# vasudeva-ram/Julia-NewtonRaphsonHANK

Hardware: AMD Instinct MI355X
Metric: sequence-space JVPs/sec (household block: BackwardIteration+ForwardIteration+aggregation, Krusell-Smith T=300) (higher is better)
Workload: dtype f64; 1 GPU; ks_2000x11_T300_N32; grid=2000x11, T=300, tangents_per_gpu=32, step=1 dual-sweep pass: primal + N tangents (hank_primal_jvp), parallelism=tangent-sharded x1

## Files before the change

### julia-newtonraphsonhank_amd/csrc/hank_device.h

```cpp
#pragma once
#include <hip/hip_runtime.h>
#include <stdint.h>
#include "hank_geom.h"

#ifndef HANK_XFWD_LQ
#define HANK_XFWD_LQ 1
#endif
#ifndef HANK_XFWD_EARLY_BATCH
#define HANK_XFWD_EARLY_BATCH 0
#endif

namespace hank {

struct Consts {
    int n_a, n_e, G, P;
    int n_hh;
    int diet;
    double beta, gamma, bc;
    const double *a, *z, *Pi;
};

struct Record {
    double *s, *kc, *A, *B, *u, *v, *pol, *lw, *ig, *Dseq;
    int *ib, *lo, *start, *clo;
    int4 *seg;
    double2 *lwg;
};

__device__ inline double wave_sum(double x) {
#pragma unroll
    for (int off = 32; off > 0; off >>= 1) x += __shfl_down(x, off, 64);
    return x;
}
__device__ inline double block_sum(double x, double *red, int nthreads) {
    const int lane = threadIdx.x & 63, wv = threadIdx.x >> 6;
    const int nw = (nthreads + 63) >> 6;
    x = wave_sum(x);
    __syncthreads();
    if (lane == 0) red[wv] = x;
    __syncthreads();
    double r = 0.0;
    if (threadIdx.x == 0)
        for (int k = 0; k < nw; k++) r += red[k];
    return r;
}
// ... 719 lines not shown
```

### julia-newtonraphsonhank_amd/csrc/hank_hip.hip

```cpp
#include "hank_kernels.h"
#include "hank_xsweep.h"
#include "hank_xspec.h"
#include "hank_jacobian.h"
#include "hank_wide.h"
#include "hank_hetx.h"
#include "hank_scen.h"
#include "hank_ssbatch.h"
#include "hank_adjoint.h"
#include "hank_boundary.h"
#include "hank_ssdiff_launch.h"
#include "../../include/hank_hip.h"

#include <cstdarg>
#include <cstdio>
#include <cstdlib>
#include <cstring>
#include <initializer_list>
#include <list>
#include <mutex>
#include <new>
#include <vector>

using namespace hank;

// ... 55 lines not shown
    GraphExec &tan_fwd(bool bnd, int NX) { return g_tfwd[bnd][NX]; }
private:
    GraphExec g_tback[2], g_tfwd[2][3];
};

constexpr int XD_MAX = 4;
constexpr int XPASS_MAX = 64;
struct XPass { int n0, N, D, groups; size_t dpol_off; };
struct XTan {
    int N = 0;
    std::vector<XPass> passes;
    DevBuf<double> dxhh, dxr, dxw, dxt;
    DevBuf<double> dpol;
    DevBuf<double> daggpart;
    DevBuf<double> dagg_pass;
    DevBuf<double> dagg_cm;
};
struct XWork {
    bool ready = false;
    int grid = 0, Sact = 0, maxt = 768, dmax = XD_MAX;
    DevBuf<XSync> sync;
    DevBuf<double> st_s, st_ds, st_D, st_dD;
    DevBuf<double> Dvirt, aggpart, rho;
    DevBuf<double> D0own;
    DevBuf<int> srcB, srcF;
    DevBuf<int2> unitsF;
    DevBuf<int> unit_overflow;
    int ucap = 64;
    bool rng_valid = false;
    DevBuf<int2> stageU;
    DevBuf<int4> stageM;
    bool front = true;
    int front_poison = 0;
    bool neigh = true;
    bool syncwave = true;
    int lds_max = 65536;
    int fault_where = 7;
    int fault = 0;
    bool src_valid = false;
    std::list<XTan> tans;
    int last_blocks = 0;
    int xspec = XSPEC_CRRA;
    int inst[4] = {-1, -1, -1, -1};
};

struct WTan {
    int N = 0;
    DevBuf<double> dxhh;
    DevBuf<double> dpol;
    DevBuf<double> dagg_cm;
};

struct CotWork {
    int N = 0;
    int V = 1;
    AdjGeom g{};
    DevBuf<double> ybar;
    DevBuf<double> yb0, yb1;
    DevBuf<double> ybx;
    DevBuf<double> st[2];
    DevBuf<double> pbar;
    DevBuf<double> partS, partM;
    DevBuf<double> xbar;
    GraphExec g_A, g_B;
    GraphExec g_AX[2];
    DevBuf<double> bnd_vbar, bnd_dbar;
// ... 587 lines not shown

static int x_setup(hank_ctx *ctx) {
    XWork &X = ctx->xw;
    if (X.ready) return HANK_OK;
    const Consts &c = ctx->c;
    hipDeviceProp_t prop;
    HIPC(ctx, hipGetDeviceProperties(&prop, ctx->device));
    X.grid = (prop.multiProcessorCount / XG) * XG;
    X.Sact = (c.n_a + XRW - 1) / XRW;
    X.maxt = 64 * (c.n_e + 1) <= 768 ? 768 : 1024;
    X.dmax = X.maxt == 768 ? XD_MAX : 2;
    const size_t G = c.G, GV = G + 64 * (size_t)c.n_e, P = c.P;
    HIPC(ctx, X.sync.alloc((size_t)2 + 2 * XPASS_MAX));
    HIPC(ctx, hipMemsetAsync(X.sync, 0, sizeof(XSync) * ((size_t)2 + 2 * XPASS_MAX), ctx->stream));
    HIPC(ctx, X.st_s.alloc(2 * XG * G));
    HIPC(ctx, X.st_ds.alloc(2 * XG * G * X.dmax));
    const size_t GM = (size_t)c.n_e * X.Sact * 64;
    HIPC(ctx, X.st_D.alloc(2 * XG * std::max(GV, GM)));
    HIPC(ctx, X.st_dD.alloc(2 * XG * GM * xslots(X.dmax + 1).SP));
    HIPC(ctx, X.Dvirt.alloc(P * c.n_e * 64));
    HIPC(ctx, X.D0own.alloc(P * c.n_e));
    HIPC(ctx, X.aggpart.alloc(2 * P * (size_t)X.Sact));
    HIPC(ctx, X.rho.alloc(P));
    HIPC(ctx, X.srcB.alloc(P * X.Sact));
    HIPC(ctx, X.srcF.alloc(P * X.Sact));
    HIPC(ctx, X.unitsF.alloc(P * X.Sact * XUCAP));
    HIPC(ctx, X.unit_overflow.alloc(1));
    HIPC(ctx, hipMemsetAsync(X.unit_overflow, 0, sizeof(int), ctx->stream));
    if (X.front && ctx->rec_lq) {
        HIPC(ctx, X.stageU.alloc(P * X.Sact * c.n_e * XU_ROWS));
        HIPC(ctx, X.stageM.alloc(P * X.Sact * c.n_e));
    }
    if (const char *ng = getenv("HANK_XNEIGH")) X.neigh = atoi(ng) != 0;
    if (const char *uc = getenv("HANK_XUCAP")) X.ucap = std::min(XUCAP, std::max(1, atoi(uc)));
    {
        double ms = 20.0;
        if (const char *wm = getenv("HANK_XWAIT_MS")) ms = atof(wm);
        const unsigned long long ticks = (unsigned long long)(std::max(ms, 0.01) * 1e5);
        HIPC(ctx, hipMemcpyToSymbol(HIP_SYMBOL(hank::g_xwait_ticks), &ticks, sizeof(ticks)));
    }
    if (const char *sv = getenv("HANK_XSYNCWAVE")) X.syncwave = atoi(sv) != 0;
    X.lds_max = (int)prop.sharedMemPerBlock;
    if (const char *xf = getenv("HANK_XFAULT")) {
        X.fault = strncmp(xf, "placement", 9) == 0 ? XERR_PLACEMENT : (strncmp(xf, "timeout", 7) == 0 ? XERR_TIMEOUT : (strncmp(xf, "stall", 5) == 0 ? 3 : 0));
        const char *w = strchr(xf, ':');
        X.fault_where = !w ? 7 : (strcmp(w, ":primal") == 0 ? 1 : (strcmp(w, ":tangent") == 0 ? 2 : (strcmp(w, ":fixedpoint") == 0 ? 4 : 7)));
    }
    HIPC(ctx, hipMemsetAsync(X.Dvirt, 0, sizeof(double) * P * c.n_e * 64, ctx->stream));
    X.ready = true;
    return HANK_OK;
}

static int x_build_tan(hank_ctx *ctx, XTan &w) {
    XWork &X = ctx->xw;
    const Consts &c = ctx->c;
    const size_t P = c.P, G = c.G;
    const int N = w.N;
    size_t off = 0;
    for (int n0 = 0; n0 < N; n0 += XG * X.dmax) {
        XPass ps;
        ps.n0 = n0; ps.N = std::min(N - n0, XG * X.dmax);
        ps.D = 1; while (XG * ps.D < ps.N) ps.D *= 2;
        ps.groups = (ps.N + ps.D - 1) / ps.D;
        ps.dpol_off = off;
        off += P * ps.groups * G * ps.D;
        w.passes.push_back(ps);
// ... 21 lines not shown
}

template <typename F>
static void x_by_maxt(const XWork &X, F launch) { if (X.maxt == 768) launch(std::integral_constant<int, 768>()); else launch(std::integral_constant<int, 1024>()); }
#define XL(...) hipLaunchKernelGGL((__VA_ARGS__), dim3(X.grid), x_block(X, c), lds, sec.stream(), a)
static bool x_has_dual_back(const XWork &X) { return X.maxt == 768; }
static void x_launch_dual_back(XSection &sec, XWork &X, const Consts &c, int D, const XDualBackArgs &a) {
    const size_t lds = x_lds_dual_back(c, D);
    if (!x_has_dual_back(X)) return;
    const XSpec sp = x_spec(X.xspec, c.n_e, c.gamma, c.diet);
    X.inst[0] = sp.ne; X.inst[1] = sp.crra;
    if (!sp.ne && !sp.crra) {
        if (D == 1) XL(k_xdual_back<1, 768>);
        else if (D == 2) XL(k_xdual_back<2, 768>);
        else XL(k_xdual_back<4, 768>);
        return;
    }
    auto by_d = [&](auto ne, auto crra) {
        constexpr int NE = decltype(ne)::value, CRRA = decltype(crra)::value;
        if (D == 1) XL(k_xdual_back<1, 768, NE, CRRA>);
        else if (D == 2) XL(k_xdual_back<2, 768, NE, CRRA>);
        else XL(k_xdual_back<4, 768, NE, CRRA>);
    };
    auto by_crra = [&](auto ne) {
        if (sp.crra) by_d(ne, std::integral_constant<int, 1>()); else if constexpr (decltype(ne)::value != 0) by_d(ne, std::integral_constant<int, 0>());
    };
    if (sp.ne == 4) by_crra(std::integral_constant<int, 4>());
    else if (sp.ne == 7) by_crra(std::integral_constant<int, 7>());
    else if (sp.ne == 11) by_crra(std::integral_constant<int, 11>());
    else by_crra(std::integral_constant<int, 0>());
}
static bool x_fwd_serves_lq(const XWork &X, const Consts &c, int D) {
#if HANK_XFWD_LQ
    return D > 0 && x_lds_fwd_lq(c, D) <= (size_t)X.lds_max;
#else
    return false;
#endif
}
static void x_launch_fwd(XSection &sec, XWork &X, const Consts &c, int D, bool val, const XSweepFwdArgs &a) {
    if (val && D > 0) { X.inst[2] = 0; X.inst[3] = 0; }
#if HANK_XFWD_LQ
    if (val && x_fwd_serves_lq(X, c, D)) {
        const size_t lds = x_lds_fwd_lq(c, D);
        x_by_maxt(X, [&](auto mt) {
            constexpr int MT = decltype(mt)::value;
            if (D == 1) XL(k_xfwd<1, true, MT, true>);
            else if (D == 2) XL(k_xfwd<2, true, MT, true>);
            else if (D == 4) { if constexpr (MT == 768) XL(k_xfwd<4, true, MT, true>); }
        });
        return;
    }
#endif
    const size_t lds = x_lds_fwd(c, D, val || D == 0);
    x_by_maxt(X, [&](auto mt) {
        constexpr int MT = decltype(mt)::value;
        if (D == 0) XL(k_xfwd<0, true, MT>);
        else if (D == 1) { if (val) XL(k_xfwd<1, true, MT>); else XL(k_xfwd<1, false, MT>); }
        else if (D == 2) { if (val) XL(k_xfwd<2, true, MT>); else XL(k_xfwd<2, false, MT>); }
        else if (D == 4) { if constexpr (MT == 768) { if (val) XL(k_xfwd<4, true, MT>); else XL(k_xfwd<4, false, MT>); } }
    });
}
static void x_launch_primal_back(XSection &sec, const XWork &X, const Consts &c, const XBackArgs &a) { const size_t lds = x_lds_primal_back(c); x_by_maxt(X, [&](auto mt) { XL(k_xprimal_back<decltype(mt)::value>); }); }
static void x_launch_tan_back(XSection &sec, const XWork &X, const Consts &c, int D, const XTanBackArgs &a) {
    const size_t lds = x_lds_tan_back(c, D);
    x_by_maxt(X, [&](auto mt) {
        constexpr int MT = decltype(mt)::value;
        if (D == 1) XL(k_xtan_back<1, MT>);
// ... 2474 lines not shown
```

### julia-newtonraphsonhank_amd/csrc/hank_xlds.h

```cpp
#pragma once
#include <cstddef>

#ifdef __HIPCC__
#define XLDS_HD __host__ __device__
#else
#define XLDS_HD
#endif

namespace hank {

constexpr size_t XCTL_BYTES = 64;

template <int D> struct XTileT { static constexpr int SL = D == 4 ? 6 : (D == 8 ? 10 : D); };
XLDS_HD inline int xtile_sl(int D) { return D == 1 ? XTileT<1>::SL : (D == 2 ? XTileT<2>::SL : XTileT<4>::SL); }

template <int NSL> struct XSlots {
    static constexpr int SP = NSL == 1 ? 1 : ((NSL + 1) / 2) * 2;
    static constexpr int SL = NSL <= 2 ? NSL : (NSL <= 6 ? 6 : 10);
};
struct XSlotsRt { int SP, SL; };
template <int NSL> constexpr XSlotsRt xslots_of() { return {XSlots<NSL>::SP, XSlots<NSL>::SL}; }
XLDS_HD inline XSlotsRt xslots(int NSL) { return NSL == 1 ? xslots_of<1>() : NSL == 2 ? xslots_of<2>() : NSL == 3 ? xslots_of<3>() : NSL == 4 ? xslots_of<4>() : xslots_of<5>(); }

struct XLdsCursor { unsigned o; size_t bytes; };
// ... 42 lines not shown
struct XLdsDualBack { unsigned tile, ash, xsh, dxsh, ctl; size_t bytes; };
XLDS_HD inline XLdsDualBack xlds_dual_back(int n_e, int n_a, int P, int D) {
    XLdsCursor o = {0, 0}; XLdsDualBack L;
    L.tile = xlds_take(o, (size_t)xslots(D + 1).SL * n_e * 64, 8);
    L.ash = xlds_take(o, ((size_t)n_a + 1) & ~(size_t)1, 8);
    L.xsh = xlds_take(o, 4 * (size_t)P, 8);
    L.dxsh = xlds_take(o, 3 * (size_t)P * D + ((n_a + 1) & 1), 8);
    return xlds_end(L, o);
}

struct XLdsFwd { unsigned tile, aggsh, Pish, closh, srcsh, ctl; size_t bytes; };
XLDS_HD inline XLdsFwd xlds_fwd(int n_e, int P, int D, bool val) {
    const int NSL = D + (val ? 1 : 0), NAP = 2 * NSL;
    XLdsCursor o = {0, 0}; XLdsFwd L;
    L.tile = xlds_take(o, (size_t)xslots(NSL).SL * n_e * 64, 8);
    L.aggsh = xlds_take(o, (size_t)n_e * 64 * NAP, 8);
    L.Pish = xlds_take(o, (size_t)n_e * n_e + 1, 8);
    L.closh = xlds_take(o, (size_t)P * n_e, 4);
    L.srcsh = xlds_take(o, P, 4);
    return xlds_end(L, o);
}

struct XLdsFwdLq { unsigned tile, aggsh, Pish, closh, srcsh, iga, ctl; size_t bytes; };
XLDS_HD inline XLdsFwdLq xlds_fwd_lq(int n_e, int n_a, int P, int D) {
    const XLdsFwd F = xlds_fwd(n_e, P, D, true);
    XLdsFwdLq L;
    L.tile = F.tile; L.aggsh = F.aggsh; L.Pish = F.Pish; L.closh = F.closh; L.srcsh = F.srcsh;
    XLdsCursor o = {F.ctl, F.bytes - XCTL_BYTES};
    xlds_take(o, (16 - F.ctl % 16) % 16, 1);
    L.iga = xlds_take(o, n_a, 8);
    return xlds_end(L, o);
}

}
```

### julia-newtonraphsonhank_amd/csrc/hank_xsweep.h

```cpp
#pragma once
#include "hank_kernels.h"
#include "hank_xaddr.h"
#include "hank_xlds.h"
#include "hank_xunits.h"
#include <type_traits>

namespace hank {

constexpr int XG = 8;
constexpr int XRW = 63;
enum { XERR_TIMEOUT = 1, XERR_PLACEMENT = 2 };
__device__ unsigned long long g_xwait_ticks = 2000000ull;
struct XDeadline {
    unsigned long long t0;
    __device__ __forceinline__ XDeadline() : t0(__builtin_amdgcn_s_memrealtime()) {}
    __device__ __forceinline__ bool expired(unsigned spins) const { return (spins & 63u) == 63u && __builtin_amdgcn_s_memrealtime() - t0 > g_xwait_ticks; }
    __device__ __forceinline__ unsigned waited_us() const { return (unsigned)((__builtin_amdgcn_s_memrealtime() - t0) / 100ull); }
};

struct XSync {
    unsigned ticket[XG][32];
    unsigned total[32];
    unsigned flag[XG][64][32];
    unsigned status[32];
// ... 375 lines not shown
        for (int q = 0; q < NS; q++) out[q] = p * v[q];
    }
    int k = 1;
    constexpr int U = 5;
    for (; k + U <= ne; k += U) {
        double v[U][SL], p[U];
#pragma unroll
        for (int u = 0; u < U; u++) { rd(k + u, v[u]); p[u] = P[(k + u) * ps]; }
        __builtin_amdgcn_sched_barrier(0);
#pragma unroll
        for (int u = 0; u < U; u++) acc(p[u], v[u]);
    }
#pragma unroll 1
    for (; k < ne; k++) {
        double v[SL];
        rd(k, v);
        acc(P[k * ps], v);
    }
}

template <int SL, int NS, bool FMA = false, bool BRK = false, int NK = 16>
__device__ __forceinline__ void xtile_mix_reg(const double *tl, const double (&pr)[NK], int ne, double *out) {
    const int ks = 64 * SL;
#pragma unroll
    for (int k = 0; k < NK; k++) {
        if (BRK && k > 0 && k >= ne) break;
        if (BRK || k < ne) {
            double v[SL];
            if (SL == 1) v[0] = tl[(size_t)k * ks];
            else {
#pragma unroll
                for (int q = 0; q < (NS + 1) / 2; q++) { const double2 d = reinterpret_cast<const double2 *>(tl + (size_t)k * ks)[q]; v[2 * q] = d.x; v[2 * q + 1] = d.y; }
            }
#pragma unroll
            for (int q = 0; q < NS; q++) out[q] = k == 0 ? pr[k] * v[q] : (FMA ? __builtin_fma(pr[k], v[q], out[q]) : out[q] + pr[k] * v[q]);
        }
    }
}

__device__ __forceinline__ void xstage_prices(double *xsh, const Consts &c, const double *xhh, const double *rho, int P) {
    for (int k = threadIdx.x; k < P; k += blockDim.x) {
        xsh[4 * k] = xhh[c.n_hh * k]; xsh[4 * k + 1] = xhh[c.n_hh * k + 1]; xsh[4 * k + 2] = hh_tr(c, xhh, k); xsh[4 * k + 3] = rho[k];
    }
}
template <int D>
__device__ __forceinline__ void xstage_dx(double *dxsh, const Consts &c, const double *dxr, const double *dxw, const double *dxt, int Ntot, int n0, int N, int x, int P) {
    for (int k = threadIdx.x; k < P * D; k += blockDim.x) {
        const int t_ = k / D, d_ = k - t_ * D;
        const bool on = x * D + d_ < N;
        const size_t ix = (size_t)t_ * Ntot + n0 + x * D + d_;
        dxsh[(t_ * 3 + 0) * D + d_] = on ? dxr[ix] : 0.0;
        dxsh[(t_ * 3 + 1) * D + d_] = on ? dxw[ix] : 0.0;
        dxsh[(t_ * 3 + 2) * D + d_] = (on && c.n_hh > 2) ? dxt[ix] : 0.0;
    }
}

struct XRecOff {
    const char *rec;
    unsigned bytes;
    unsigned pol, ib, A, B, u, v, s, kc, lo, lw, ig, Dseq;
    unsigned lq;
};
static_assert(sizeof(XRecOff) == 64, "XRecOff: a field more moves the arguments behind it in k_xdual_back and k_xfwd");

struct XBackArgs {
    Consts c;
// ... 583 lines not shown
    const double *D0;
    const double *dpol;
    int groups;
    double *Dvirt;
    double *aggpart;
    double *daggpart;
    const int *src;
    const int *overflow;
    const int2 *units;
    int all_members;
    XRecOff ro;
    unsigned dpol_bytes;
    unsigned iga;
};

#if HANK_XFWD_LQ
template <int D, bool VAL, int MAXT, bool LQ = false>
#else
template <int D, bool VAL, int MAXT>
#endif
__global__ void __launch_bounds__(MAXT) k_xfwd(XSweepFwdArgs A) {
#pragma clang fp contract(fast)
#if !HANK_XFWD_LQ
    constexpr bool LQ = false;
#endif
    constexpr int NSL = D + (VAL ? 1 : 0);
    constexpr int SP = XSlots<NSL>::SP, SL = XSlots<NSL>::SL;
    constexpr int IV = D;
    constexpr int DD = D > 0 ? D : 1;
    constexpr bool PIREG = NSL < 4;
    constexpr bool XB = VAL && D > 0;
    constexpr bool EARLYB = XB && HANK_XFWD_EARLY_BATCH != 0;
    static_assert(!LQ || XB, "the packed record is read through the record's descriptor");
    extern __shared__ __attribute__((aligned(16))) double xl[];
    const Consts &c = A.c;
    const Record &R = A.R;
    const int ne = c.n_e, na = c.n_a, P = c.P, G = c.G;
    const XLdsFwd L = xlds_fwd(ne, P, D, VAL);
    double *tile = xlds_at<double>(xl, L.tile), *Pish = xlds_at<double>(xl, L.Pish), *aggsh = xlds_at<double>(xl, L.aggsh);
    constexpr int NAP = 2 * NSL;
    int *closh = xlds_at<int>(xl, L.closh), *srcsh = xlds_at<int>(xl, L.srcsh), *ctl = xlds_at<int>(xl, L.ctl);
    double *igash = nullptr;
    if constexpr (LQ) { const XLdsFwdLq Q = xlds_fwd_lq(ne, na, P, D); igash = xlds_at<double>(xl, Q.iga); ctl = xlds_at<int>(xl, Q.ctl); }
    (void)igash;
    if (*A.overflow) return;
    const XMember mb = xmember_join(A.sy, ctl, A.groups, na);
    if (!mb.on) return;
    const int x = mb.x, cW = mb.c, Sact = mb.Sact;
    constexpr bool RECL = VAL && D == 0;
    const bool recD = VAL && x == 0, recL = RECL && x == 1 % A.groups;
    for (int k = threadIdx.x; k < ne * ne; k += blockDim.x) Pish[k] = c.Pi[k];
    for (int k = threadIdx.x; k < P * ne; k += blockDim.x) closh[k] = R.clo[k];
    if constexpr (LQ) { for (int k = threadIdx.x; k < na; k += blockDim.x) igash[k] = reinterpret_cast<const double *>(A.ro.rec + A.iga)[k]; }
    for (int k = threadIdx.x; k < P; k += blockDim.x) {
        int w = A.src[(size_t)k * Sact + cW];
        if (A.all_members || (recL && ((w >> 17) & 1))) w = (w & ~0xffff) | ((Sact - 1) << 8);
        srcsh[k] = w;
    }
    const XRoles rl = xroles(ne);
    const int lane = rl.lane, wv = rl.wv, e = rl.e; const bool syncw = rl.syncw, sync_duty = rl.sync_duty;
    const int r0 = cW * XRW, r = r0 + lane;
    const bool own = !syncw && lane < XRW && r < na;
    const bool virt = !syncw && lane == 63;
    const bool live = own || virt;
    const size_t pt = (size_t)e * na + (own ? r : 0);
    const double xar = c.a[own ? r : 0];
    const size_t GM = (size_t)ne * Sact * 64;
    const size_t gx = (size_t)x * GM;
    const size_t slot = gx + ((size_t)e * Sact + cW) * 64 + lane;
    const size_t hs = (size_t)XG * GM;
    double pr[16];
#pragma unroll
    for (int k = 0; k < 16; k++) pr[k] = (PIREG && k < ne) ? c.Pi[ne * e + k] : 0.0;
    XRows<SP> rows;
    const int iGM = ne * Sact * 64;
    if constexpr (XB) rows.init_buf(A.st, 2 * XG * iGM); else rows.init(A.st, 2 * hs);
    __amdgpu_buffer_rsrc_t rrec, rdp;
    if constexpr (XB) { rrec = buf_rsrc(A.ro.rec, A.ro.bytes); rdp = buf_rsrc(A.dpol, A.dpol_bytes); }
    const int ipt = e * na + (own ? r : 0), igx = x * iGM, ihs = XG * iGM, islot = (e * Sact + cW) * 64;
    double *const myt = tile + ((size_t)e * 64 + lane) * SL;
    double mxp[NSL];
#pragma unroll
    for (int k = 0; k < NSL; k++) mxp[k] = 0.0;
    if constexpr (VAL) { if (own) mxp[IV] = A.D0[pt]; }
    {
        double sv[SP];
#pragma unroll
        for (int k = 0; k < SP; k++) sv[k] = k < NSL ? mxp[k] : 0.0;
        if constexpr (XB) { if (live) rows.store_vs(lane, igx + islot, sv); }
        else if (live) rows.store(slot, sv);
    }
    double polr = 0.0, Dr = 0.0, lwr = 0.0, igr = 0.0, dpr[DD];
#pragma unroll
    for (int k = 0; k < DD; k++) dpr[k] = 0.0;
    auto prefetch = [&](int t) {
        if constexpr (XB) {
            polr = buf_ld64<0>(rrec, ipt * 8, (int)(A.ro.pol + (unsigned)(t * G) * 8u));
            xload_row_buf<DD>(rdp, ipt * (8 * D), (int)((unsigned)((t * A.groups + x) * G) * (unsigned)(8 * D)), dpr);
            return;
        }
        const size_t ro = (size_t)t * G + (size_t)e * na + (own ? r : 0);
        polr = R.pol[ro];
        if constexpr (D > 0) xload_row_plain<DD>(A.dpol + ((size_t)t * A.groups + x) * (size_t)G * D + ((size_t)e * na + (own ? r : 0)) * D, dpr);
        if constexpr (RECL) { lwr = R.lw[ro]; igr = R.ig[ro]; }
        else if constexpr (!VAL && D > 0) Dr = R.Dseq[ro + G];
    };
    int2 ud[2];
    int qlo[2];
    double qw[2], qg[2], qdn[2], qdp[2][DD], dd[2][SP];
    bool qon[2], qvl[2];
    int qrow[2] = {0, 0};
    int qfl[2] = {1, 1};
    (void)qfl;
    const int2 *const ubase = A.units + (size_t)cW * XUCAP;
    auto unit_ld = [&](int tu, int u) -> int2 {
        return A.units[(unsigned)((tu * Sact + cW) * XUCAP + u)];
    };
    auto unit_desc = [&](int t, int u) -> int2 {
        int2 q;
        if constexpr (XB) q = unit_ld(t, u); else q = ubase[(size_t)t * Sact * XUCAP + u];
        return make_int2(__builtin_amdgcn_readfirstlane(q.x), __builtin_amdgcn_readfirstlane(q.y));
    };
    auto load_rec = [&](auto U, int t, int2 d, int i0) {
        constexpr int u = decltype(U)::value;
        const int ue = d.x & 15, ja = (d.x >> 4) & 0xfff, cnt = (d.x >> 16) & 0xfff, nv = (d.y >> 16) & 0xff;
        const int i = i0 + lane;
        const bool real = i < cnt;
        qvl[u] = !real && i < cnt + nv;
        qon[u] = real || qvl[u];
        const size_t cb = (size_t)t * G + (size_t)ue * na;
        const int j = real ? ja + i : (qvl[u] ? 0 : min(ja + max(cnt - 1, 0), na - 1));
        if constexpr (XB) {
            const int icb = t * G + ue * na;
            qrow[u] = qvl[u] ? (i - cnt) * 64 + 63 : (real ? (j / XRW) * 64 + j % XRW : 0);
            if constexpr (LQ) {
                const xv4u q = __builtin_amdgcn_raw_buffer_load_b128(rrec, j * 16, (int)(A.ro.lq + (unsigned)icb * 16u), 0);
                qw[u] = __hiloint2double((int)q.y, (int)q.x); qlo[u] = (int)q.z; qfl[u] = (int)q.w;
            } else {
                qlo[u] = buf_ld32<0>(rrec, j * 4, (int)(A.ro.lo + (unsigned)icb * 4u));
                qw[u] = buf_ld64<0>(rrec, j * 8, (int)(A.ro.lw + (unsigned)icb * 8u));
                qg[u] = buf_ld64<0>(rrec, j * 8, (int)(A.ro.ig + (unsigned)icb * 8u));
            }
            xload_row_buf<DD>(rdp, j * (8 * D), (int)((unsigned)((t * A.groups + x) * G + ue * na) * (unsigned)(8 * D)), qdp[u]);
            return;
        }
        qlo[u] = R.lo[cb + j];
        if constexpr (VAL) qw[u] = R.lw[cb + j];
        else { const double2 wg = R.lwg[cb + j]; qw[u] = wg.x; qg[u] = wg.y; if constexpr (D > 0) qdn[u] = R.Dseq[cb + G + j]; }
        if constexpr (D > 0) xload_row_plain<DD>(A.dpol + (((size_t)t * A.groups + x) * G + (size_t)ue * na + j) * D, qdp[u]);
    };
    auto load_state = [&](auto U, size_t hb, int hc, int2 d, int i0) {
        constexpr int u = decltype(U)::value;
        const int ue = d.x & 15, ja = (d.x >> 4) & 0xfff, cnt = (d.x >> 16) & 0xfff;
#pragma unroll
        for (int k = 0; k < SP; k++) dd[u][k] = 0.0;
        const int i = i0 + lane, j = ja + i;
        if constexpr (XB) {
            rows.load_vs(qrow[u], hc * ihs + igx + ue * Sact * 64, dd[u]);
            return;
        }
        const size_t row = qvl[u] ? ((size_t)ue * Sact + (i - cnt)) * 64 + 63 : ((size_t)ue * Sact + j / XRW) * 64 + j % XRW;
        if (qon[u]) rows.load(hb + gx + row, dd[u]);
    };
    auto set_g = [&](auto U) {
        constexpr int u = decltype(U)::value;
        if constexpr (LQ) { const double g = igash[min((unsigned)qlo[u], (unsigned)(na - 1))]; qg[u] = (qfl[u] & 1) ? 0.0 : g; }
    };
    const std::integral_constant<int, 0> I0;
    const std::integral_constant<int, 1> I1;
    int2 udn[2];
    bool udv[2] = {false, false};
    udn[0] = udn[1] = make_int2(0, 0);
    auto request_units = [&](int t) {
        const int tc = min(t, P - 1);
        int nu = (srcsh[tc] >> 18) & 0xff;
        nu = t < P ? nu : 0;
        udv[0] = wv < nu; udv[1] = wv + ne < nu;
        if constexpr (XB) { udn[0] = unit_ld(tc, udv[0] ? wv : 0); udn[1] = unit_ld(tc, udv[1] ? wv + ne : 0); }
        else {
            udn[0] = ubase[(size_t)tc * Sact * XUCAP + (udv[0] ? wv : 0)];
            udn[1] = ubase[(size_t)tc * Sact * XUCAP + (udv[1] ? wv + ne : 0)];
        }
    };
    auto take_units = [&]() {
        ud[0] = udv[0] ? make_int2(__builtin_amdgcn_readfirstlane(udn[0].x), __builtin_amdgcn_readfirstlane(udn[0].y)) : make_int2(0, 0);
        ud[1] = udv[1] ? make_int2(__builtin_amdgcn_readfirstlane(udn[1].x), __builtin_amdgcn_readfirstlane(udn[1].y)) : make_int2(0, 0);
    };
    constexpr int DPI = D == 0 ? 0 : (D <= 2 ? 1 : D / 2);
    constexpr int XFWD_NLD = 1 + DPI + (RECL ? 2 : ((!VAL && D > 0) ? 1 : 0));
// ... 20 lines not shown
            double v[NAP];
            if (NAP == 1) v[0] = ap[(size_t)k2 * 64 * NAP];
            else {
#pragma unroll
                for (int q = 0; q < NAP / 2; q++) { const double2 d = reinterpret_cast<const double2 *>(ap + (size_t)k2 * 64 * NAP)[q]; v[2 * q] = d.x; v[2 * q + 1] = d.y; }
            }
#pragma unroll
            for (int k = 0; k < NAP; k++) sk[k] += v[k];
        }
        const size_t pb = (size_t)tp * Sact + cW;
#pragma unroll
        for (int k = 0; k < D; k++) {
            const double pd = xwave_reduce63(sk[k]), pd2 = xwave_reduce63(sk[NSL + k]);
            if (lane == 63) { A.daggpart[pb * (size_t)(2 * XG * D) + x * D + k] = pd; A.daggpart[pb * (size_t)(2 * XG * D) + XG * D + x * D + k] = pd2; }
        }
        if constexpr (VAL) {
            if (recD) {
                const double pD = xwave_reduce63(sk[IV]), pD2 = xwave_reduce63(sk[NSL + IV]);
                if (lane == 63) { A.aggpart[2 * pb] = pD; A.aggpart[2 * pb + 1] = pD2; }
            }
        }
    };
    for (int t = 0; t < P; t++) {
        XSTAMP(1, son, t, 0);
        const size_t base = (size_t)t * G + (size_t)e * na;
        const size_t hb = (size_t)cur * hs;
        const int sw = srcsh[t];
        int clo = 0;
        if (!syncw) {
            clo = min(max(closh[t * ne + e], 0), na);
            double z[SL];
#pragma unroll
            for (int k = 0; k < SL; k++) z[k] = 0.0;
            xtile_store<SL>(myt, z);
            set_g(I0);
            set_g(I1);
        }
        if (sync_duty) xpoll(A.sy, x, sw & 255, (sw >> 8) & 255, (unsigned)(t + 1));
        xlds_barrier();
        XSTAMP(1, son, t, 1);
        if (sync_duty && t > 0) reduce_agg(t - 1);
        double pagg[DD];
#pragma unroll
        for (int k = 0; k < DD; k++) pagg[k] = 0.0;
        double v0 = 0.0;
        if (!syncw) {
            const bool need0 = recL && r0 == 0 && vnz && clo == 0;
            if constexpr (RECL) {
                if (need0 && lane < Sact) v0 = rows.load_one(hb + gx + ((size_t)e * Sact + lane) * 64 + 63, IV);
            }
            load_state(I0, hb, cur, ud[0], 0);
            load_state(I1, hb, cur, ud[1], 0);
            auto process_pc = [&](auto U, int2 d) {
                constexpr int u = decltype(U)::value;
                const int ta = d.y & 0xff, tb = (d.y >> 8) & 0xff;
                double *const colt = tile + (size_t)(d.x & 15) * 64 * SL;
                const double w = qw[u], w1 = 1.0 - w;
                double gD = qg[u], Dv = 0.0;
                if constexpr (VAL) { Dv = dd[u][IV]; gD = qg[u] * Dv; }
                else { if (qvl[u]) gD = 0.0; }
                const int tl = qlo[u] - r0, th = tl + 1;
                const bool doL = qon[u] && tl >= ta && tl < tb, doH = qon[u] && th >= ta && th < tb;
                const int thp = __builtin_amdgcn_update_dpp(-2, doH ? th : -2, 0x138, 0xf, 0xf, false);
                const bool take = doL && thp == tl;
                const bool given = __builtin_amdgcn_update_dpp(0, take ? 1 : 0, 0x130, 0xf, 0xf, false) != 0;
                double *const tpl = colt + (size_t)(doL ? tl : 0) * SL, *const tph = colt + (size_t)(doH ? th : 0) * SL;
#pragma unroll
                for (int k = 0; k < D; k++) {
                    const double hk = w * dd[u][k] + gD * qdp[u][k];
                    const double hp = xdpp<0x138, 0xf, 0xf>(hk);
                    const double lk = w1 * dd[u][k] - gD * qdp[u][k];
                    if (doL) lds_add(tpl + k, take ? lk + hp : lk);
                    if (doH && !given) lds_add(tph + k, hk);
                }
                if constexpr (VAL) {
                    if (doL) lds_add(tpl + IV, w1 * Dv);
                    if (doH) lds_add(tph + IV, w * Dv);
                }
                if constexpr (!VAL) {
                    if (doL && !qvl[u]) {
#pragma unroll
                        for (int k = 0; k < D; k++) pagg[k] += qdp[u][k] * qdn[u];
                    }
                }
            };
            auto process_1 = [&](auto U, int2 d) {
                constexpr int u = decltype(U)::value;
                if (!qon[u]) return;
                const int ta = d.y & 0xff, tb = (d.y >> 8) & 0xff;
                double *const colt = tile + (size_t)(d.x & 15) * 64 * SL;
                const double w = qw[u], w1 = 1.0 - w;
                double gD = qg[u], Dv = 0.0;
                if constexpr (VAL) { Dv = dd[u][IV]; gD = qg[u] * Dv; }
                else { if (qvl[u]) gD = 0.0; }
                const int tl = qlo[u] - r0, th = tl + 1;
                if (tl >= ta && tl < tb) {
                    double *tp = colt + (size_t)tl * SL;
#pragma unroll
                    for (int k = 0; k < D; k++) lds_add(tp + k, w1 * dd[u][k] - gD * qdp[u][k]);
                    if constexpr (VAL) lds_add(tp + IV, w1 * Dv);
                    if constexpr (!VAL) {
                        if (!qvl[u]) {
#pragma unroll
                            for (int k = 0; k < D; k++) pagg[k] += qdp[u][k] * qdn[u];
                        }
                    }
                }
                if (th >= ta && th < tb) {
                    double *tp = colt + (size_t)th * SL;
#pragma unroll
                    for (int k = 0; k < D; k++) lds_add(tp + k, w * dd[u][k] + gD * qdp[u][k]);
                    if constexpr (VAL) lds_add(tp + IV, w * Dv);
                }
            };
            constexpr bool PRECOMB = NSL >= 3;
            auto process = [&](auto U, int2 d) { if constexpr (PRECOMB) process_pc(U, d); else process_1(U, d); };
            process(I0, ud[0]);
            process(I1, ud[1]);
            const int nu = (sw >> 18) & 0xff;
            for (int u2 = wv; u2 < nu; u2 += ne) {
                const int2 d = u2 < 2 * ne ? ud[u2 >= ne ? 1 : 0] : unit_desc(t, u2);
                const int tot = ((d.x >> 16) & 0xfff) + ((d.y >> 16) & 0xff);
                for (int i0 = u2 < 2 * ne ? 64 : 0; i0 < tot; i0 += 64) {
                    load_rec(I0, t, d, i0);
                    load_state(I0, hb, cur, d, i0);
                    set_g(I0);
                    process(I0, d);
                }
            }
            if constexpr (RECL) { if (need0) v0 = xwave_sum(v0); }
            take_units();
            if constexpr (EARLYB) next_units_loads(t);
            XSTAMP(1, son, t, 2);
            double cT[NSL];
#pragma unroll
            for (int k = 0; k < NSL; k++) cT[k] = ((own && r < clo) || (virt && clo > 0 && vnz)) ? mxp[k] : 0.0;
            if (clo > r0) {
#pragma unroll
                for (int k = 0; k < NSL; k++) cT[k] = xwave_reduce63(cT[k]);
            }
            if (virt) xtile_store_n<SL, NSL>(myt, cT);
        }
        XSTAMP(1, son, t, 3);
        XSTAMPV(1, son, t);
        if (sync_duty) xpoll(A.sy, x, 0, Sact - 1, (unsigned)(t + 1));
        xlds_barrier();
        XSTAMP(1, son, t, 4);
        vnz = ((sw >> 16) & 1) != 0;
        const int nxt = cur ^ 1;
        if (!syncw) {
            if constexpr (!EARLYB) next_units_loads(t);
            double mx[NSL];
            if (PIREG) xtile_mix_reg<SL, NSL, true>(tile + (size_t)lane * SL, pr, ne, mx);
            else xtile_mix<SL, NSL, true>(tile + (size_t)lane * SL, Pish + ne * e, 1, ne, mx);
            if (live) {
                double sv[SP];
#pragma unroll
                for (int k = 0; k < SP; k++) sv[k] = k < NSL ? mx[k] : 0.0;
                if constexpr (XB) rows.store_vs(lane, nxt * ihs + igx + islot, sv);
                else rows.store((size_t)nxt * hs + slot, sv);
            }
            double at[NAP];
#pragma unroll
            for (int k = 0; k < NAP; k++) at[k] = 0.0;
            if constexpr (RECL) {
                if (recL && own) {
                    double Dfull = mxp[IV];
                    if (r == 0 && clo == 0) Dfull += v0;
                    R.lwg[base + r] = make_double2(lwr, igr * Dfull);
                }
            }
            if constexpr (VAL) {
                if (recD) {
                    if (own) {
                        if constexpr (XB) buf_st64<0>(mx[IV], rrec, ipt * 8, (int)(A.ro.Dseq + (unsigned)((t + 1) * G) * 8u));
                        else R.Dseq[(size_t)(t + 1) * G + pt] = mx[IV];
                    } else if (virt) A.Dvirt[((size_t)t * ne + e) * 64 + cW] = mx[IV];
                    at[IV] = live ? polr * mx[IV] : 0.0;
                    at[NSL + IV] = live ? xar * mx[IV] : 0.0;
                }
            }
#pragma unroll
            for (int k = 0; k < D; k++) {
                double term = live ? polr * mx[k] : 0.0;
                if constexpr (VAL) term = live ? (polr * mx[k] + dpr[k] * mx[IV]) : 0.0;
                else term = (term + pagg[k]) + ((own && r < clo) ? dpr[k] * Dr : 0.0);
                at[k] = term;
                at[NSL + k] = live ? xar * mx[k] : 0.0;
            }
            xtile_store<NAP>(aggsh + ((size_t)e * 64 + lane) * NAP, at);
#pragma unroll
            for (int k = 0; k < NSL; k++) mxp[k] = mx[k];
        }
        cur = nxt;
        XSTAMP(1, son, t, 5);
        if (!syncw) {
            asm volatile("; XFWD_BATCH_BEGIN" ::: "memory");
            prefetch(min(t + 1, P - 1));
            XSTAMP(1, son, t, 7);
            asm volatile("; XFWD_BATCH_END\n\ts_waitcnt vmcnt(%0)" ::"n"(XFWD_NLD) : "memory");
            XSTAMP(1, son, t, 8);
        }
        xlds_barrier();
        if (sync_duty) xpublish(A.sy, x, cW, (unsigned)(t + 2));
        XSTAMP(1, son, t, 6);
    }
    if (sync_duty) reduce_agg(P - 1);
}
static inline size_t x_lds_fwd(const Consts &c, int D, bool val) { return xlds_fwd(c.n_e, c.P, D, val).bytes; }
static inline size_t x_lds_fwd_lq(const Consts &c, int D) { return xlds_fwd_lq(c.n_e, c.n_a, c.P, D).bytes; }

__global__ void k_xunits_fwd(Consts c, Record R, int Sact, int *src, int2 *units, int *overflow, int ucap) {
    __shared__ int2 su[16][XUCAP];
    __shared__ int scnt[16], slo, shi, sany0;
    __shared__ int sst[16][XRW + 3];
    const int t = blockIdx.x, m = blockIdx.y, ne = c.n_e, na = c.n_a;
    const int r0 = m * XRW, nrows = min(XRW, na - r0);
    __shared__ int sclo[16], sclop[16], soff[17];
    if (threadIdx.x == 0) { slo = m; shi = m; sany0 = 0; }
    if ((int)threadIdx.x < ne) {
        sclo[threadIdx.x] = R.clo[(size_t)t * ne + threadIdx.x];
        sclop[threadIdx.x] = t > 0 ? R.clo[(size_t)(t - 1) * ne + threadIdx.x] : 0;
    }
    for (int k = threadIdx.x; k < ne * (XRW + 3); k += blockDim.x) {
        const int e = k / (XRW + 3), q = k - e * (XRW + 3);
        sst[e][q] = min(max(R.start[((size_t)t * ne + e) * (na + 1) + min(max(r0 - 1 + q, 0), na)], 0), na);
    }
    __syncthreads();
    bool vnz = false;
    for (int e = 0; e < ne; e++) vnz = vnz || sclop[e] > 0;
    const int lane = threadIdx.x & 63, wave = threadIdx.x >> 6, nwaves = blockDim.x >> 6;
    for (int e = wave; e < ne; e += nwaves) {
        const int clo = sclo[e];
        auto S = [&](int rr) { return sst[e][min(max(rr - (r0 - 1), 0), XRW + 2)]; };
        auto lanes_of = [&](int a, int b, int *ja_out, bool *has0_out) {
            const int ja = S(r0 + a - 1 < 0 ? 0 : r0 + a - 1);
            const bool has0 = ja == 0 && clo <= 0 && vnz;
            const int cnt = max(S(r0 + b) - ja, 0);
            *ja_out = ja; *has0_out = has0;
            return cnt;
        };
// ... 274 lines not shown
```

Measured before the change: 9331 JVPs/s.

## Store forward-sweep LDS tile slot-major (SoA) for conflict-free lane access

Changes the forward-sweep LDS tile from lane-major AoS (SL doubles per lane) to a slot-major layout where each slot is a 64-lane contiguous stripe. This applies to the LQ packed-record path, covering the scatter-adds, the stores and the Pi-mix reads. The aim is to cut LDS bank conflicts from strided per-lane access in the mix and the scatter. It also adds an optional transposed lane mapping for flat units, off by default, and an env switch to turn off the packed LQ path. The SoA mix uses volatile LDS loads with a sched barrier, which may limit how the compiler schedules those loads.

```diff
diff --git a/julia-newtonraphsonhank_amd/csrc/hank_device.h b/julia-newtonraphsonhank_amd/csrc/hank_device.h
--- a/julia-newtonraphsonhank_amd/csrc/hank_device.h
+++ b/julia-newtonraphsonhank_amd/csrc/hank_device.h
@@ -9,8 +9,16 @@
 #ifndef HANK_XFWD_EARLY_BATCH
 #define HANK_XFWD_EARLY_BATCH 0
 #endif
+#ifndef HANK_XFWD_TILE_SOA
+#define HANK_XFWD_TILE_SOA 1
+#endif
+#ifndef HANK_XFWD_FLAT_TR
+#define HANK_XFWD_FLAT_TR 0
+#endif
 
 namespace hank {
+
+constexpr int XFLAT_NUM = 3, XFLAT_DEN = 2;
 
 struct Consts {
     int n_a, n_e, G, P;
diff --git a/julia-newtonraphsonhank_amd/csrc/hank_hip.hip b/julia-newtonraphsonhank_amd/csrc/hank_hip.hip
--- a/julia-newtonraphsonhank_amd/csrc/hank_hip.hip
+++ b/julia-newtonraphsonhank_amd/csrc/hank_hip.hip
@@ -111,6 +111,7 @@
     DevBuf<int4> stageM;
     bool front = true;
     int front_poison = 0;
+    bool packed = true;
     bool neigh = true;
     bool syncwave = true;
     int lds_max = 65536;
@@ -764,6 +765,7 @@
         HIPC(ctx, X.stageM.alloc(P * X.Sact * c.n_e));
     }
     if (const char *ng = getenv("HANK_XNEIGH")) X.neigh = atoi(ng) != 0;
+    if (const char *pk = getenv("HANK_XFWD_PACKED")) X.packed = atoi(pk) != 0;
     if (const char *uc = getenv("HANK_XUCAP")) X.ucap = std::min(XUCAP, std::max(1, atoi(uc)));
     {
         double ms = 20.0;
@@ -851,7 +853,7 @@
 }
 static bool x_fwd_serves_lq(const XWork &X, const Consts &c, int D) {
 #if HANK_XFWD_LQ
-    return D > 0 && x_lds_fwd_lq(c, D) <= (size_t)X.lds_max;
+    return X.packed && D > 0 && x_lds_fwd_lq(c, D) <= (size_t)X.lds_max;
 #else
     return false;
 #endif
diff --git a/julia-newtonraphsonhank_amd/csrc/hank_xlds.h b/julia-newtonraphsonhank_amd/csrc/hank_xlds.h
--- a/julia-newtonraphsonhank_amd/csrc/hank_xlds.h
+++ b/julia-newtonraphsonhank_amd/csrc/hank_xlds.h
@@ -98,4 +98,10 @@
     return xlds_end(L, o);
 }
 
+constexpr int XTILE_SOA_SLOT = 64;
+XLDS_HD inline unsigned xtile_soa_at(int NSL, int col, int slot, int lane) {
+    return (unsigned)(((col * NSL + slot) * XTILE_SOA_SLOT + lane) * 8);
 }
+XLDS_HD inline size_t xtile_soa_bytes(int n_e, int NSL) { return (size_t)n_e * NSL * XTILE_SOA_SLOT * 8; }
+
+}
diff --git a/julia-newtonraphsonhank_amd/csrc/hank_xsweep.h b/julia-newtonraphsonhank_amd/csrc/hank_xsweep.h
--- a/julia-newtonraphsonhank_amd/csrc/hank_xsweep.h
+++ b/julia-newtonraphsonhank_amd/csrc/hank_xsweep.h
@@ -431,6 +431,64 @@
 #pragma unroll
                 for (int q = 0; q < (NS + 1) / 2; q++) { const double2 d = reinterpret_cast<const double2 *>(tl + (size_t)k * ks)[q]; v[2 * q] = d.x; v[2 * q + 1] = d.y; }
             }
+#pragma unroll
+            for (int q = 0; q < NS; q++) out[q] = k == 0 ? pr[k] * v[q] : (FMA ? __builtin_fma(pr[k], v[q], out[q]) : out[q] + pr[k] * v[q]);
+        }
+    }
+}
+
+typedef const volatile __attribute__((address_space(3))) double xlds_cvdouble;
+__device__ __forceinline__ double xtile_soa_ld(const double *p) { return *(xlds_cvdouble *)p; }
+template <int NS>
+__device__ __forceinline__ void xtile_soa_store(double *t, const double *v) {
+#pragma unroll
+    for (int q = 0; q < NS; q++) t[q * XTILE_SOA_SLOT] = v[q];
+}
+template <int NS, bool FMA = false>
+__device__ __forceinline__ void xtile_soa_mix(const double *tl, const double *P, int ps, int ne, double *out) {
+    constexpr int ks = XTILE_SOA_SLOT * NS;
+    auto rd = [&](int k, double *v) {
+#pragma unroll
+        for (int q = 0; q < NS; q++) v[q] = xtile_soa_ld(tl + (size_t)k * ks + q * XTILE_SOA_SLOT);
+    };
+    auto acc = [&](double p, const double *v) {
+#pragma unroll
+        for (int q = 0; q < NS; q++) out[q] = FMA ? __builtin_fma(p, v[q], out[q]) : out[q] + p * v[q];
+    };
+    {
+        double v[NS];
+        rd(0, v);
+        const double p = P[0];
+#pragma unroll
+        for (int q = 0; q < NS; q++) out[q] = p * v[q];
+    }
+    int k = 1;
+    constexpr int U = 5;
+    for (; k + U <= ne; k += U) {
+        double v[U][NS], p[U];
+#pragma unroll
+        for (int u = 0; u < U; u++) { rd(k + u, v[u]); p[u] = P[(k + u) * ps]; }
+        __builtin_amdgcn_sched_barrier(0);
+#pragma unroll
+        for (int u = 0; u < U; u++) acc(p[u], v[u]);
+    }
+#pragma unroll 1
+    for (; k < ne; k++) {
+        double v[NS];
+        rd(k, v);
+        acc(P[k * ps], v);
+    }
+}
+template <int NS, bool FMA = false, bool BRK = false, int NK = 16>
+__device__ __forceinline__ void xtile_soa_mix_reg(const double *tl, const double (&pr)[NK], int ne, double *out) {
+    constexpr int ks = XTILE_SOA_SLOT * NS;
+#pragma unroll
+    for (int k = 0; k < NK; k++) {
+        if (BRK && k > 0 && k >= ne) break;
+        if (BRK || k < ne) {
+            double v[NS];
+#pragma unroll
+            for (int q = 0; q < NS; q++) v[q] = tl[(size_t)k * ks + q * XTILE_SOA_SLOT];
 #pragma unroll
             for (int q = 0; q < NS; q++) out[q] = k == 0 ? pr[k] * v[q] : (FMA ? __builtin_fma(pr[k], v[q], out[q]) : out[q] + pr[k] * v[q]);
         }
@@ -1080,6 +1138,18 @@
     constexpr bool XB = VAL && D > 0;
     constexpr bool EARLYB = XB && HANK_XFWD_EARLY_BATCH != 0;
     static_assert(!LQ || XB, "the packed record is read through the record's descriptor");
+#if HANK_XFWD_TILE_SOA
+    constexpr bool SOA = LQ;
+    constexpr int TCS = SOA ? XTILE_SOA_SLOT * NSL : 64 * SL;
+    static_assert(NSL <= SL, "the slot-major tile lies inside the tile piece");
+#define XT_COL(c) (SOA ? tile + (size_t)(c) * (XTILE_SOA_SLOT * NSL) : tile + (size_t)(c) * 64 * SL)
+#define XT_ROW(p, r) (SOA ? (p) + (size_t)(r) : (p) + (size_t)(r) * SL)
+#define XT_SLOT(p, k) (SOA ? (p) + (k) * XTILE_SOA_SLOT : (p) + (k))
+#else
+#define XT_COL(c) (tile + (size_t)(c) * 64 * SL)
+#define XT_ROW(p, r) ((p) + (size_t)(r) * SL)
+#define XT_SLOT(p, k) ((p) + (k))
+#endif
     extern __shared__ __attribute__((aligned(16))) double xl[];
     const Consts &c = A.c;
     const Record &R = A.R;
@@ -1126,7 +1196,11 @@
     __amdgpu_buffer_rsrc_t rrec, rdp;
     if constexpr (XB) { rrec = buf_rsrc(A.ro.rec, A.ro.bytes); rdp = buf_rsrc(A.dpol, A.dpol_bytes); }
     const int ipt = e * na + (own ? r : 0), igx = x * iGM, ihs = XG * iGM, islot = (e * Sact + cW) * 64;
+#if HANK_XFWD_TILE_SOA
+    double *const myt = SOA ? tile + (size_t)e * TCS + lane : tile + ((size_t)e * 64 + lane) * SL;
+#else
     double *const myt = tile + ((size_t)e * 64 + lane) * SL;
+#endif
     double mxp[NSL];
 #pragma unroll
     for (int k = 0; k < NSL; k++) mxp[k] = 0.0;
@@ -1169,10 +1243,21 @@
         if constexpr (XB) q = unit_ld(t, u); else q = ubase[(size_t)t * Sact * XUCAP + u];
         return make_int2(__builtin_amdgcn_readfirstlane(q.x), __builtin_amdgcn_readfirstlane(q.y));
     };
+#if HANK_XFWD_FLAT_TR
+    const int ltr = (lane & 15) * 4 + (lane >> 4);
+    auto unit_flat = [&](int2 d) -> bool {
+        const int cnt = (d.x >> 16) & 0xfff, ta = d.y & 0xff, tb = (d.y >> 8) & 0xff;
+        return XFLAT_DEN * cnt > XFLAT_NUM * (tb - ta);
+    };
+    auto unit_lane = [&](int2 d) -> int { return unit_flat(d) ? ltr : lane; };
+#define XUNIT_LANE(d) unit_lane(d)
+#else
+#define XUNIT_LANE(d) lane
+#endif
     auto load_rec = [&](auto U, int t, int2 d, int i0) {
         constexpr int u = decltype(U)::value;
         const int ue = d.x & 15, ja = (d.x >> 4) & 0xfff, cnt = (d.x >> 16) & 0xfff, nv = (d.y >> 16) & 0xff;
-        const int i = i0 + lane;
+        const int i = i0 + XUNIT_LANE(d);
         const bool real = i < cnt;
         qvl[u] = !real && i < cnt + nv;
         qon[u] = real || qvl[u];
@@ -1202,7 +1287,7 @@
         const int ue = d.x & 15, ja = (d.x >> 4) & 0xfff, cnt = (d.x >> 16) & 0xfff;
 #pragma unroll
         for (int k = 0; k < SP; k++) dd[u][k] = 0.0;
-        const int i = i0 + lane, j = ja + i;
+        const int i = i0 + XUNIT_LANE(d), j = ja + i;
         if constexpr (XB) {
             rows.load_vs(qrow[u], hc * ihs + igx + ue * Sact * 64, dd[u]);
             return;
@@ -1289,6 +1374,9 @@
             double z[SL];
 #pragma unroll
             for (int k = 0; k < SL; k++) z[k] = 0.0;
+#if HANK_XFWD_TILE_SOA
+            if constexpr (SOA) xtile_soa_store<NSL>(myt, z); else
+#endif
             xtile_store<SL>(myt, z);
             set_g(I0);
             set_g(I1);
@@ -1311,7 +1399,7 @@
             auto process_pc = [&](auto U, int2 d) {
                 constexpr int u = decltype(U)::value;
                 const int ta = d.y & 0xff, tb = (d.y >> 8) & 0xff;
-                double *const colt = tile + (size_t)(d.x & 15) * 64 * SL;
+                double *const colt = XT_COL(d.x & 15);
                 const double w = qw[u], w1 = 1.0 - w;
                 double gD = qg[u], Dv = 0.0;
                 if constexpr (VAL) { Dv = dd[u][IV]; gD = qg[u] * Dv; }
@@ -1319,20 +1407,24 @@
                 const int tl = qlo[u] - r0, th = tl + 1;
                 const bool doL = qon[u] && tl >= ta && tl < tb, doH = qon[u] && th >= ta && th < tb;
                 const int thp = __builtin_amdgcn_update_dpp(-2, doH ? th : -2, 0x138, 0xf, 0xf, false);
+#if HANK_XFWD_FLAT_TR
+                const bool take = doL && thp == tl && !unit_flat(d);
+#else
                 const bool take = doL && thp == tl;
+#endif
                 const bool given = __builtin_amdgcn_update_dpp(0, take ? 1 : 0, 0x130, 0xf, 0xf, false) != 0;
-                double *const tpl = colt + (size_t)(doL ? tl : 0) * SL, *const tph = colt + (size_t)(doH ? th : 0) * SL;
+                double *const tpl = XT_ROW(colt, doL ? tl : 0), *const tph = XT_ROW(colt, doH ? th : 0);
 #pragma unroll
                 for (int k = 0; k < D; k++) {
                     const double hk = w * dd[u][k] + gD * qdp[u][k];
                     const double hp = xdpp<0x138, 0xf, 0xf>(hk);
                     const double lk = w1 * dd[u][k] - gD * qdp[u][k];
-                    if (doL) lds_add(tpl + k, take ? lk + hp : lk);
-                    if (doH && !given) lds_add(tph + k, hk);
+                    if (doL) lds_add(XT_SLOT(tpl, k), take ? lk + hp : lk);
+                    if (doH && !given) lds_add(XT_SLOT(tph, k), hk);
                 }
                 if constexpr (VAL) {
-                    if (doL) lds_add(tpl + IV, w1 * Dv);
-                    if (doH) lds_add(tph + IV, w * Dv);
+                    if (doL) lds_add(XT_SLOT(tpl, IV), w1 * Dv);
+                    if (doH) lds_add(XT_SLOT(tph, IV), w * Dv);
                 }
                 if constexpr (!VAL) {
                     if (doL && !qvl[u]) {
@@ -1345,17 +1437,17 @@
                 constexpr int u = decltype(U)::value;
                 if (!qon[u]) return;
                 const int ta = d.y & 0xff, tb = (d.y >> 8) & 0xff;
-                double *const colt = tile + (size_t)(d.x & 15) * 64 * SL;
+                double *const colt = XT_COL(d.x & 15);
                 const double w = qw[u], w1 = 1.0 - w;
                 double gD = qg[u], Dv = 0.0;
                 if constexpr (VAL) { Dv = dd[u][IV]; gD = qg[u] * Dv; }
                 else { if (qvl[u]) gD = 0.0; }
                 const int tl = qlo[u] - r0, th = tl + 1;
                 if (tl >= ta && tl < tb) {
-                    double *tp = colt + (size_t)tl * SL;
-#pragma unroll
-                    for (int k = 0; k < D; k++) lds_add(tp + k, w1 * dd[u][k] - gD * qdp[u][k]);
-                    if constexpr (VAL) lds_add(tp + IV, w1 * Dv);
+                    double *tp = XT_ROW(colt, tl);
+#pragma unroll
+                    for (int k = 0; k < D; k++) lds_add(XT_SLOT(tp, k), w1 * dd[u][k] - gD * qdp[u][k]);
+                    if constexpr (VAL) lds_add(XT_SLOT(tp, IV), w1 * Dv);
                     if constexpr (!VAL) {
                         if (!qvl[u]) {
 #pragma unroll
@@ -1364,10 +1456,10 @@
                     }
                 }
                 if (th >= ta && th < tb) {
-                    double *tp = colt + (size_t)th * SL;
-#pragma unroll
-                    for (int k = 0; k < D; k++) lds_add(tp + k, w * dd[u][k] + gD * qdp[u][k]);
-                    if constexpr (VAL) lds_add(tp + IV, w * Dv);
+                    double *tp = XT_ROW(colt, th);
+#pragma unroll
+                    for (int k = 0; k < D; k++) lds_add(XT_SLOT(tp, k), w * dd[u][k] + gD * qdp[u][k]);
+                    if constexpr (VAL) lds_add(XT_SLOT(tp, IV), w * Dv);
                 }
             };
             constexpr bool PRECOMB = NSL >= 3;
@@ -1396,6 +1488,9 @@
 #pragma unroll
                 for (int k = 0; k < NSL; k++) cT[k] = xwave_reduce63(cT[k]);
             }
+#if HANK_XFWD_TILE_SOA
+            if constexpr (SOA) { if (virt) xtile_soa_store<NSL>(myt, cT); } else
+#endif
             if (virt) xtile_store_n<SL, NSL>(myt, cT);
         }
         XSTAMP(1, son, t, 3);
@@ -1408,6 +1503,12 @@
         if (!syncw) {
             if constexpr (!EARLYB) next_units_loads(t);
             double mx[NSL];
+#if HANK_XFWD_TILE_SOA
+            if constexpr (SOA) {
+                if (PIREG) xtile_soa_mix_reg<NSL, true>(tile + lane, pr, ne, mx);
+                else xtile_soa_mix<NSL, true>(tile + lane, Pish + ne * e, 1, ne, mx);
+            } else
+#endif
             if (PIREG) xtile_mix_reg<SL, NSL, true>(tile + (size_t)lane * SL, pr, ne, mx);
             else xtile_mix<SL, NSL, true>(tile + (size_t)lane * SL, Pish + ne * e, 1, ne, mx);
             if (live) {
@@ -1464,6 +1565,10 @@
     }
     if (sync_duty) reduce_agg(P - 1);
 }
+#undef XUNIT_LANE
+#undef XT_COL
+#undef XT_ROW
+#undef XT_SLOT
 static inline size_t x_lds_fwd(const Consts &c, int D, bool val) { return xlds_fwd(c.n_e, c.P, D, val).bytes; }
 static inline size_t x_lds_fwd_lq(const Consts &c, int D) { return xlds_fwd_lq(c.n_e, c.n_a, c.P, D).bytes; }
 
```

Result: faster. 9551 JVPs/s, median of 6 (+2.4%).
